# jaxonwang/k-mer-count

Hardware: AMD Instinct MI355X
Metric: k-mers/sec (whole node) on synthetic FASTA, k=31; counts bit-exact vs ref (higher is better)
Workload: dtype u64; 1 GPU; 10 GB synthetic FASTA (random_fasta_generator.py distribution, seed 2, pool 10), k=31, canonical, 1xMI355X; records_per_gpu=22371032, bases_per_gpu=8948412800, kmers_per_gpu=8277281840, kmers_all_gpus=8277281840, distinct=3350, algo=walk

## Files before the change

k-mer-count_amd/csrc/kmc_extract.hip.h:

```cpp
#pragma once
#include "kmc_stream.hip.h"
#include "kmc_msd.hip.h"

template <int KW> struct ExtractLds {
    u32 sbits[KMC_STREAM_WAVES][64];
    alignas(16) u64 tr[KMC_STREAM_WAVES][KW == 1 ? 256 : 512];
    u32 hist[KMC_MSD_NB + 3];
    u64 s_or[KMC_STREAM_WAVES][2], s_and[KMC_STREAM_WAVES][2];
};

__device__ __forceinline__ void extract_store_half(u64* tr, int lane, const u64 (&v)[8], u64* __restrict__ out_chunk, int h) {
    typedef unsigned long long u64x2_t __attribute__((ext_vector_type(2)));
#pragma unroll
    for (int q = 0; q < 4; ++q) {
        u64x2_t p = {v[2 * q], v[2 * q + 1]};
        *reinterpret_cast<u64x2_t*>(&tr[lane * 8 + 2 * ((q + (lane >> 1)) & 3)]) = p;
    }
    __builtin_amdgcn_fence(__ATOMIC_RELEASE, "wavefront");
    __builtin_amdgcn_wave_barrier();
    __builtin_amdgcn_fence(__ATOMIC_ACQUIRE, "wavefront");
    u64 x[8];
#pragma unroll
    for (int i = 0; i < 8; ++i) {
        const int l = 8 * i + (lane >> 3), j = lane & 7;
        x[i] = tr[l * 8 + 2 * (((j >> 1) + (l >> 1)) & 3) + (j & 1)];
    }
    __builtin_amdgcn_fence(__ATOMIC_RELEASE, "wavefront");
    __builtin_amdgcn_wave_barrier();
    __builtin_amdgcn_fence(__ATOMIC_ACQUIRE, "wavefront");
#pragma unroll
    for (int i = 0; i < 8; ++i) out_chunk[16 * (8 * i + (lane >> 3)) + 8 * h + (lane & 7)] = x[i];
}

template <int KW, bool CANON>
__global__ __launch_bounds__(KMC_STREAM_THREADS)
void kmc_extract_hist_kernel(const uint8_t* __restrict__ bases, u64 n_bases, const u64* __restrict__ offsets, u64 n_reads, int k,
                             u64 chunk_begin, u64 chunk_end, u64 range_begin, u32 n_ranges, u64* __restrict__ counters,
                             u64* __restrict__ out_hi, u64* __restrict__ out_lo, u32* __restrict__ hist, u32 hist_r0,
                             u64* __restrict__ rand_, u64* __restrict__ ror_) {
    constexpr int NW = 2 * KW + 1;
    extern __shared__ __align__(16) unsigned char extract_smem[];
    ExtractLds<KW>& L = *reinterpret_cast<ExtractLds<KW>*>(extract_smem);
    const int tid = threadIdx.x, lane = tid & 63, wv = tid >> 6;
    const int kb = 2 * k;
    const ChunkKeys<KW> K(k);
    const int dshift = kb > KMC_MSD_BITS ? kb - KMC_MSD_BITS : 0;
    const u32 dmask = kb >= KMC_MSD_BITS ? (u32)KMC_MSD_ND - 1u : (1u << kb) - 1u;
    u64 nk = 0;

    for (u32 r = blockIdx.x; r < n_ranges; r += gridDim.x) {
        __syncthreads();
        for (u32 d = tid; d < KMC_MSD_NB; d += KMC_STREAM_THREADS) L.hist[d] = 0;
        __syncthreads();
        u64 a_lo = ~0ull, a_hi = ~0ull, o_lo = 0, o_hi = 0;
        const u64 c0 = chunk_begin + (u64)r * (KMC_MSD_RANGE / KMC_CHUNK) + 4u * (u64)wv, c1 = c0 + 4;
        const u64 cfirst = c0 > 0 ? c0 - 1 : 0;
        ChunkWalk W(offsets, n_reads, cfirst, lane);
        for (u64 c = cfirst; c < c1; ++c) {
            W.step(bases, n_bases, c, c < chunk_end, L.sbits[wv]);
            if (c >= c0) {
                u32 X[NW], Yp[NW + 1];
                u32 inv16 = chunk_windows<KW>(W, k, X);
                if (W.pp < range_begin) {
                    const u64 nskip = range_begin - W.pp;
                    inv16 |= nskip >= 16 ? 0xFFFFu : ((1u << (u32)nskip) - 1u);
                }
                chunk_rc_stream<KW, CANON>(K, X, Yp);
                const u64 obase = W.cb - chunk_begin * KMC_CHUNK;
                auto key_at = [&](int j, u64& khi, u64& klo) -> bool {
                    chunk_key<KW, CANON>(K, X, Yp, j, khi, klo);
                    const bool ok = !((inv16 >> j) & 1);
                    const u32 d = ok ? (msd_bits<KW>(khi, klo, dshift) & dmask) : (u32)KMC_MSD_ND;
                    atomicAdd(&L.hist[d], 1u);
                    if (ok) {
                        a_lo &= klo; o_lo |= klo;
                        if constexpr (KW == 2) { a_hi &= khi; o_hi |= khi; }
                    } else {
                        klo = ~0ull; khi = ~0ull;
                    }
                    return ok;
                };
                if constexpr (KW == 1) {
                    u64 vlo[16];
#pragma unroll
                    for (int j = 0; j < 16; ++j) { u64 khi; nk += key_at(j, khi, vlo[j]) ? 1u : 0u; }
                    stream_store_transposed(reinterpret_cast<u32*>(L.tr[wv]), lane, vlo, out_lo + obase);
                } else {
#pragma unroll
                    for (int h = 0; h < 2; ++h) {
                        u64 vlo[8], vhi[8];
#pragma unroll
                        for (int j = 0; j < 8; ++j) nk += key_at(8 * h + j, vhi[j], vlo[j]) ? 1u : 0u;
                        extract_store_half(L.tr[wv], lane, vlo, out_lo + obase, h);
                        extract_store_half(L.tr[wv], lane, vhi, out_hi + obase, h);
                    }
                }
            }
        }
#pragma unroll
        for (int o = 32; o > 0; o >>= 1) {
            a_lo &= __shfl_xor(a_lo, o); o_lo |= __shfl_xor(o_lo, o);
            if (KW == 2) { a_hi &= __shfl_xor(a_hi, o); o_hi |= __shfl_xor(o_hi, o); }
        }
        if (lane == 0) { L.s_and[wv][0] = a_hi; L.s_and[wv][1] = a_lo; L.s_or[wv][0] = o_hi; L.s_or[wv][1] = o_lo; }
        __syncthreads();
        for (u32 d = tid; d < KMC_MSD_NB; d += KMC_STREAM_THREADS) hist[msd_hist_idx((size_t)hist_r0 + r, d)] = L.hist[d];
        if (tid == 0) {
            u64 ah = ~0ull, al = ~0ull, oh = 0, ol = 0;
            for (int w = 0; w < KMC_STREAM_WAVES; ++w) { ah &= L.s_and[w][0]; al &= L.s_and[w][1]; oh |= L.s_or[w][0]; ol |= L.s_or[w][1]; }
            if (KW == 1) { ah = 0; oh = 0; }
            if (KW == 1 && al == ~0ull && ol == 0) { ah = ~0ull; }
            rand_[2 * (size_t)r] = ah; rand_[2 * (size_t)r + 1] = al;
            ror_[2 * (size_t)r] = oh; ror_[2 * (size_t)r + 1] = ol;
        }
    }
    nk = wave_sum_u64(nk);
    if (lane == 0 && nk) atomicAdd((unsigned long long*)&counters[KMC_CTR_KMERS], nk);
}
```

k-mer-count_amd/csrc/kmc_msd.hip.h:

```cpp
#pragma once
#include <type_traits>
#include "kmc_device.hip.h"
#include "kmc_scan.hip.h"

#define KMC_MSD_RANGE 65536
static inline unsigned msd_range_for(unsigned long long n) {
    unsigned r = 4096;
    while (r < KMC_MSD_RANGE && (unsigned long long)r * 2048 < n) r <<= 1;
    return r;
}
#define KMC_MSD_BITS 10
#define KMC_MSD_ND (1 << KMC_MSD_BITS)
#define KMC_MSD_NB (KMC_MSD_ND + 1)
#define KMC_MSD_THREADS 256
#define KMC_MSD_LEAF1 2048
#ifndef KMC_MSD_LEAF2
#define KMC_MSD_LEAF2 2048
#endif
#define KMC_MSD_LEAF2W 1024
#ifndef KMC_MSD_THREAD_SORT
#define KMC_MSD_THREAD_SORT 32
#endif
#ifndef KMC_MSD_LEAF_LOGNSB
#define KMC_MSD_LEAF_LOGNSB 9
#endif
#define KMC_MSD_LEAF_NSB (1 << KMC_MSD_LEAF_LOGNSB)

struct MsdSeg { u32 begin, len, hib, parity; };
__device__ __forceinline__ int msd_seg_shift(u32 hib) { return hib > KMC_MSD_BITS ? (int)hib - KMC_MSD_BITS : 0; }
__device__ __forceinline__ u32 msd_seg_mask(u32 hib) { return hib >= KMC_MSD_BITS ? (u32)KMC_MSD_ND - 1u : (1u << hib) - 1u; }
struct MsdTerm { u32 begin, len, kind, parity; };
#define KMC_MSD_CNT_BITS 14

struct MsdCtl {
    u32 n_next;
    u32 n_term;
    u32 n_valid;
    u32 n_ranges;
    u32 overflow;
    u32 n_pairs;
    u32 scan_total;
    u32 pad;
    unsigned long long w_total;
    u32 n_cnt;
    u32 n_cnt2;
    u32 n_dups[64];
};

__host__ __device__ __forceinline__ size_t msd_hist_idx(size_t r, u32 d) { return ((r >> 6) * KMC_MSD_NB + d) * 64 + (r & 63); }
static inline size_t msd_hist_words(size_t n_ranges) { return ((n_ranges + 63) / 64) * 64 * (size_t)KMC_MSD_NB; }

template <int KW>
__device__ __forceinline__ bool msd_is_filler(u64 hi, u64 lo, int kb) {
    if (KW == 1) return kb < 64 && (lo >> kb) != 0;
    return (hi >> (kb - 64)) != 0;
}
template <int KW>
__device__ __forceinline__ u32 msd_bits(u64 hi, u64 lo, int shift) {
    if (KW == 1) return (u32)(lo >> shift);
    if (shift >= 64) return (u32)(hi >> (shift - 64));
    if (shift == 0) return (u32)lo;
    return (u32)((lo >> shift) | (hi << (64 - shift)));
}

__global__ __launch_bounds__(1024)
void kmc_msd_ranges_kernel(const MsdSeg* __restrict__ seg, u32 n_seg, u32 rsz, u32* __restrict__ first, MsdCtl* ctl) {
    __shared__ u32 part[1024];
    const u32 tid = threadIdx.x;
    const u32 per = (n_seg + 1023) / 1024;
    const u32 a = min(tid * per, n_seg), b = min(a + per, n_seg);
    u32 s = 0;
    for (u32 i = a; i < b; ++i) s += (seg[i].len + rsz - 1) / rsz;
    part[tid] = s;
    __syncthreads();
    for (u32 o = 1; o < 1024; o <<= 1) {
        u32 v = tid >= o ? part[tid - o] : 0;
        __syncthreads();
        part[tid] += v;
        __syncthreads();
    }
    u32 run = tid ? part[tid - 1] : 0;
    for (u32 i = a; i < b; ++i) { first[i] = run; run += (seg[i].len + rsz - 1) / rsz; }
    if (tid == 1023) { first[n_seg] = part[1023]; ctl->n_ranges = part[1023]; }
}

__device__ __forceinline__ u32 msd_seg_of(const u32* __restrict__ first, u32 n_seg, u32 r) {
    u32 lo = 0, hi = n_seg;
    while (hi - lo > 1) {
        const u32 mid = (lo + hi) >> 1;
        if (first[mid] <= r) lo = mid; else hi = mid;
    }
    return lo;
}

template <int KW>
__global__ __launch_bounds__(KMC_MSD_THREADS)
void kmc_msd_hist_kernel(const u64* __restrict__ hi0, const u64* __restrict__ lo0, const u64* __restrict__ hi1, const u64* __restrict__ lo1,
                         const MsdSeg* __restrict__ seg, u32 n_seg,
                         const u32* __restrict__ first, u32 rsz, int kb, int level0,
                         u32* __restrict__ hist, u64* __restrict__ rmin, u64* __restrict__ rmax, const MsdCtl* __restrict__ ctl) {
    __shared__ u32 h[4][KMC_MSD_NB + 3];
    __shared__ u64 smin[4][2], smax[4][2];
    const u32 r = blockIdx.x, tid = threadIdx.x, wv = tid >> 6;
    if (r >= ctl->n_ranges) return;
    for (u32 i = tid; i < 4 * (KMC_MSD_NB + 3); i += KMC_MSD_THREADS) (&h[0][0])[i] = 0;
    __syncthreads();
    const u32 s = msd_seg_of(first, n_seg, r);
    const u32 idx = r - first[s];
    const u32 b = seg[s].begin + idx * rsz;
    const u32 n = min(rsz, seg[s].len - idx * rsz);
    const int shift = msd_seg_shift(seg[s].hib);
    const u32 mask = msd_seg_mask(seg[s].hib);
    const u64* const khi = seg[s].parity ? hi1 : hi0;
    const u64* const klo = seg[s].parity ? lo1 : lo0;
    u64 mnh = ~0ull, mnl = ~0ull, mxh = 0, mxl = 0;
    for (u32 i = tid; i < n; i += KMC_MSD_THREADS) {
        const u64 lo = klo[b + i], hi = KW == 2 ? khi[b + i] : 0ull;
        u32 d;
        if (level0 && msd_is_filler<KW>(hi, lo, kb)) d = KMC_MSD_ND;
        else {
            d = msd_bits<KW>(hi, lo, shift) & mask;
            if (key_less(hi, lo, mnh, mnl)) { mnh = hi; mnl = lo; }
            if (key_less(mxh, mxl, hi, lo)) { mxh = hi; mxl = lo; }
        }
        atomicAdd(&h[wv][d], 1u);
    }
#pragma unroll
    for (int o = 32; o > 0; o >>= 1) {
        const u64 oh = __shfl_xor(mnh, o), ol = __shfl_xor(mnl, o);
        if (key_less(oh, ol, mnh, mnl)) { mnh = oh; mnl = ol; }
        const u64 ph = __shfl_xor(mxh, o), pl = __shfl_xor(mxl, o);
        if (key_less(mxh, mxl, ph, pl)) { mxh = ph; mxl = pl; }
    }
    if ((tid & 63) == 0) { smin[wv][0] = mnh; smin[wv][1] = mnl; smax[wv][0] = mxh; smax[wv][1] = mxl; }
    __syncthreads();
    for (u32 d = tid; d < KMC_MSD_NB; d += KMC_MSD_THREADS) hist[msd_hist_idx(r, d)] = h[0][d] + h[1][d] + h[2][d] + h[3][d];
    if (tid == 0) {
        for (int w = 1; w < 4; ++w) {
            if (key_less(smin[w][0], smin[w][1], mnh, mnl)) { mnh = smin[w][0]; mnl = smin[w][1]; }
            if (key_less(mxh, mxl, smax[w][0], smax[w][1])) { mxh = smax[w][0]; mxl = smax[w][1]; }
        }
        rmin[2 * (size_t)r] = mnh; rmin[2 * (size_t)r + 1] = mnl;
        rmax[2 * (size_t)r] = mxh; rmax[2 * (size_t)r + 1] = mxl;
    }
}

__global__ __launch_bounds__(KMC_MSD_THREADS)
void kmc_msd_scan_a_kernel(u32 n_seg, u32 S, const u32* __restrict__ first, u32* __restrict__ hist, u32* __restrict__ stot) {
    const u32 s = blockIdx.x / S, j = blockIdx.x % S, lane = threadIdx.x & 63, wv = threadIdx.x >> 6;
    if (s >= n_seg) return;
    const u32 r0 = first[s], r1 = first[s + 1];
    if (r1 - r0 == 1) return;
    for (u32 d = j * 4 + wv; d < KMC_MSD_NB; d += 4 * S) {
        u32 run = 0;
        for (u32 base = r0; base < r1; base += 256) {
            u32 v[4];
#pragma unroll
            for (int u = 0; u < 4; ++u) {
                const u32 r = base + 64u * u + lane;
                v[u] = r < r1 ? hist[msd_hist_idx(r, d)] : 0u;
            }
#pragma unroll
            for (int u = 0; u < 4; ++u) {
                const u32 r = base + 64u * u + lane;
                u32 inc = v[u];
#pragma unroll
                for (int o = 1; o < 64; o <<= 1) { const u32 t = __shfl_up(inc, o); if ((int)lane >= o) inc += t; }
                if (r < r1) hist[msd_hist_idx(r, d)] = run + inc - v[u];
                run += __shfl(inc, 63);
            }
        }
        if (lane == 0) stot[(size_t)s * KMC_MSD_NB + d] = run;
    }
}

__global__ __launch_bounds__(KMC_MSD_ND)
void kmc_msd_scan_kernel(const MsdSeg* __restrict__ seg, u32 n_seg, const u32* __restrict__ first, u32* __restrict__ hist, const u32* __restrict__ stot,
                         const u64* __restrict__ rmin, const u64* __restrict__ rmax, u32* __restrict__ cbase, u32* __restrict__ seg_skip,
                         int level0, int wide, u32 leaf_cap, u32 cnt_bits,
                         MsdSeg* __restrict__ next, u32 next_cap, MsdTerm* __restrict__ term, u32 term_cap,
                         unsigned long long* __restrict__ bitmap, MsdCtl* ctl) {
    constexpr int NWV = KMC_MSD_ND / 64;
    __shared__ u32 tot[KMC_MSD_NB + 7];
    __shared__ u32 cb_s[KMC_MSD_ND];
    __shared__ u32 wsum[NWV];
    __shared__ u64 smm[NWV][4];
    const u32 s = blockIdx.x, tid = threadIdx.x, lane = tid & 63, wv = tid >> 6;
    const u32 r0 = first[s], r1 = first[s + 1];
    {
        u64 mnh = ~0ull, mnl = ~0ull, mxh = 0, mxl = 0;
        for (u32 r = r0 + tid; r < r1; r += KMC_MSD_ND) {
            const u64 ah = rmin[2 * (size_t)r], al = rmin[2 * (size_t)r + 1], bh = rmax[2 * (size_t)r], bl = rmax[2 * (size_t)r + 1];
            if (key_less(ah, al, mnh, mnl)) { mnh = ah; mnl = al; }
            if (key_less(mxh, mxl, bh, bl)) { mxh = bh; mxl = bl; }
        }
#pragma unroll
        for (int o = 32; o > 0; o >>= 1) {
            const u64 oh = __shfl_xor(mnh, o), ol = __shfl_xor(mnl, o);
            if (key_less(oh, ol, mnh, mnl)) { mnh = oh; mnl = ol; }
            const u64 ph = __shfl_xor(mxh, o), pl = __shfl_xor(mxl, o);
            if (key_less(mxh, mxl, ph, pl)) { mxh = ph; mxl = pl; }
        }
        if (lane == 0) { smm[wv][0] = mnh; smm[wv][1] = mnl; smm[wv][2] = mxh; smm[wv][3] = mxl; }
    }
    if (r1 - r0 == 1) {
        for (u32 d = tid; d < KMC_MSD_NB; d += KMC_MSD_ND) { tot[d] = hist[msd_hist_idx(r0, d)]; hist[msd_hist_idx(r0, d)] = 0; }
    } else {
        for (u32 d = tid; d < KMC_MSD_NB; d += KMC_MSD_ND) tot[d] = stot[(size_t)s * KMC_MSD_NB + d];
    }
    __syncthreads();
    bool all_equal;
    int top_diff = -1;
    {
        u64 mnh = smm[0][0], mnl = smm[0][1], mxh = smm[0][2], mxl = smm[0][3];
        for (int w = 1; w < NWV; ++w) {
            if (key_less(smm[w][0], smm[w][1], mnh, mnl)) { mnh = smm[w][0]; mnl = smm[w][1]; }
            if (key_less(mxh, mxl, smm[w][2], smm[w][3])) { mxh = smm[w][2]; mxl = smm[w][3]; }
        }
        all_equal = mnh == mxh && mnl == mxl;
        const u64 xh = mnh ^ mxh, xl = mnl ^ mxl;
        if (xh) top_diff = 127 - __clzll((long long)xh);
        else if (xl) top_diff = 63 - __clzll((long long)xl);
    }
    const int shift = msd_seg_shift(seg[s].hib);
    const bool last_level = shift == 0;
    const u32 src_parity = seg[s].parity;
    const u32 n_filler = level0 ? tot[KMC_MSD_ND] : 0;
    const bool equal = all_equal && seg[s].len > n_filler && (!level0 || n_filler == 0);
    const u32 mine = tot[tid];
    u32 inc = mine;
#pragma unroll
    for (int o = 1; o < 64; o <<= 1) { const u32 v = __shfl_up(inc, o); if ((int)lane >= o) inc += v; }
    if (lane == 63) wsum[wv] = inc;
    __syncthreads();
    u32 wbase = 0;
    for (u32 w = 0; w < wv; ++w) wbase += wsum[w];
    const u32 cb = seg[s].begin + wbase + inc - mine;
    cbase[(size_t)s * KMC_MSD_NB + tid] = cb;
    cb_s[tid] = cb;
    __syncthreads();
    __shared__ u32 l_tb[KMC_MSD_ND], l_tl[KMC_MSD_ND], l_tk[KMC_MSD_ND], l_nb[KMC_MSD_ND], l_nl[KMC_MSD_ND];
    const bool nomove = !equal && !last_level && top_diff >= 0 && top_diff < shift && n_filler == 0;
    if (wv != 0 && (!wide || equal || nomove)) return;
    const u32 lb = wide ? wv * 64u : 0u;
    if (tid == 0) {
        cbase[(size_t)s * KMC_MSD_NB + KMC_MSD_ND] = 0;
        seg_skip[s] = (equal || nomove) ? 1u : 0u;
        if (level0) ctl->n_valid = seg[s].len - n_filler;
    }
    u32 nt = 0, nn = 0, ncnt = 0;
    u32 q_hib = (u32)shift, q_par = src_parity ^ 1u, t_par = src_parity ^ 1u;
    if (equal) {
        if (lane == 0) { l_tb[0] = seg[s].begin; l_tl[0] = seg[s].len; l_tk[0] = 1u; }
        nt = 1; t_par = src_parity;
    } else if (nomove && cnt_bits && (u32)(top_diff + 1) <= cnt_bits && seg[s].len > leaf_cap) {
        if (lane == 0) { l_tb[0] = seg[s].begin; l_tl[0] = seg[s].len; l_tk[0] = 2u | ((u32)(top_diff + 1) << 8); }
        nt = 1; ncnt = 1; t_par = src_parity;
    } else if (nomove) {
        if (lane == 0) { l_nb[0] = seg[s].begin; l_nl[0] = seg[s].len; }
        nn = 1; q_hib = (u32)(top_diff + 1); q_par = src_parity;
    } else {
        u32 gb = 0, gl = 0;
        auto flush = [&]() { if (lane == 0) { l_tb[lb + nt] = gb; l_tl[lb + nt] = gl; l_tk[lb + nt] = gl == 1 ? 1u : 0u; } ++nt; gl = 0; };
        const int jb = wide ? (int)wv : 0, je = wide ? (int)wv + 1 : NWV;
        for (int j = jb; j < je; ++j) {
            const u32 Tj = tot[j * 64 + lane], Cj = cb_s[j * 64 + lane];
            unsigned long long live = __builtin_amdgcn_ballot_w64(Tj != 0);
            while (live) {
                const int bl = (int)__builtin_ctzll(live);
                live &= live - 1;
                const u32 m = (u32)__builtin_amdgcn_readlane((int)Tj, bl);
                const u32 cbv = (u32)__builtin_amdgcn_readlane((int)Cj, bl);
                if (m > leaf_cap) {
                    if (gl) flush();
                    if (last_level) { if (lane == 0) { l_tb[lb + nt] = cbv; l_tl[lb + nt] = m; l_tk[lb + nt] = 1u; } ++nt; }
                    else if (cnt_bits && (u32)shift <= cnt_bits) {
                        if (lane == 0) { l_tb[lb + nt] = cbv; l_tl[lb + nt] = m; l_tk[lb + nt] = 2u | ((u32)shift << 8); }
                        ++nt; ++ncnt;
                    }
                    else { if (lane == 0) { l_nb[lb + nn] = cbv; l_nl[lb + nn] = m; } ++nn; }
                } else {
                    if (gl && gl + m > leaf_cap) flush();
                    if (!gl) gb = cbv;
                    gl += m;
                }
            }
        }
        if (gl) flush();
    }
    u32 t_base = 0, n_base = 0;
    if (lane == 0) {
        if (nt) { t_base = atomicAdd(&ctl->n_term, nt); if (t_base + nt > term_cap) atomicOr(&ctl->overflow, 1u); }
        if (nn) { n_base = atomicAdd(&ctl->n_next, nn); if (n_base + nn > next_cap) atomicOr(&ctl->overflow, 2u); }
        if (ncnt) atomicAdd(&ctl->n_cnt, ncnt);
    }
    t_base = (u32)__builtin_amdgcn_readfirstlane((int)t_base);
    n_base = (u32)__builtin_amdgcn_readfirstlane((int)n_base);
    __builtin_amdgcn_fence(__ATOMIC_RELEASE, "wavefront");
    __builtin_amdgcn_wave_barrier();
    __builtin_amdgcn_fence(__ATOMIC_ACQUIRE, "wavefront");
    for (u32 i = lane; i < nt; i += 64) {
        if (t_base + i >= term_cap) break;
        const u32 bg = l_tb[lb + i];
        term[t_base + i] = MsdTerm{bg, l_tl[lb + i], l_tk[lb + i], t_par};
        atomicOr(&bitmap[bg >> 6], 1ull << (bg & 63));
    }
    for (u32 i = lane; i < nn; i += 64) {
        if (n_base + i >= next_cap) break;
        next[n_base + i] = MsdSeg{l_nb[lb + i], l_nl[lb + i], q_hib, q_par};
    }
}

#ifdef KMC_LEAF_STAMPS
__device__ unsigned long long kmc_leaf_stamps[16];
#define LEAF_STAMP(i) do { __syncthreads(); if (threadIdx.x == 0) { const unsigned long long now_ = __builtin_amdgcn_s_memtime(); atomicAdd(&kmc_leaf_stamps[i], now_ - t_prev_); t_prev_ = __builtin_amdgcn_s_memtime(); } } while (0)
#else
#define LEAF_STAMP(i) do { } while (0)
#endif
template <int KW, bool WEIGHTS> struct MsdScatterLds {
    static constexpr int WORDS = KW + (WEIGHTS ? 1 : 0);
    static constexpr int TILE = WORDS == 1 ? 16384 : (WORDS == 2 ? 8192 : 4096);
    u64 lo[TILE];
    u64 hi[KW == 2 ? TILE : 1];
    u64 w[WEIGHTS ? TILE : 1];
    u32 cnt[KMC_MSD_NB + 3];
    u32 gdst[KMC_MSD_NB + 3];
    u32 cur[KMC_MSD_NB + 3];
    u32 wsum[16];
};
template <int KW, bool WEIGHTS>
__global__ __launch_bounds__(1024)
void kmc_msd_scatter_kernel(u64* __restrict__ hi0, u64* __restrict__ lo0, u64* __restrict__ w0,
                            u64* __restrict__ hi1, u64* __restrict__ lo1, u64* __restrict__ w1,
                            const MsdSeg* __restrict__ seg, u32 n_seg, const u32* __restrict__ first, u32 rsz,
                            const u32* __restrict__ hist, const u32* __restrict__ cbase, const u32* __restrict__ seg_skip,
                            int kb, int level0, const MsdCtl* __restrict__ ctl) {
    extern __shared__ __align__(16) unsigned char msd_smem[];
    typedef MsdScatterLds<KW, WEIGHTS> LT;
    LT& L = *reinterpret_cast<LT*>(msd_smem);
    constexpr int TILE = LT::TILE, PER = TILE / 1024;
    const u32 r = blockIdx.x, tid = threadIdx.x, lane = tid & 63, wv = tid >> 6;
    if (r >= ctl->n_ranges) return;
    const u32 s = msd_seg_of(first, n_seg, r);
    if (seg_skip[s]) return;
    const int shift = msd_seg_shift(seg[s].hib);
    const u32 mask = msd_seg_mask(seg[s].hib);
    const bool sp = seg[s].parity != 0;
    const u64* const khi = sp ? hi1 : hi0;
    const u64* const klo = sp ? lo1 : lo0;
    const u64* const kw = sp ? w1 : w0;
    u64* const ohi = sp ? hi0 : hi1;
    u64* const olo = sp ? lo0 : lo1;
    u64* const ow = sp ? w0 : w1;
    for (u32 d = tid; d < KMC_MSD_NB; d += 1024) L.cur[d] = cbase[(size_t)s * KMC_MSD_NB + d] + hist[msd_hist_idx(r, d)];
    const u32 idx = r - first[s];
    const u32 b = seg[s].begin + idx * rsz;
    const u32 n = min(rsz, seg[s].len - idx * rsz);
    static_assert(PER % 2 == 0, "keys per thread must be even");
    typedef unsigned long long u64x2_t __attribute__((ext_vector_type(2)));
    const u32 off = b & 1u;
    u64 nlo[PER], nhi[PER], nw[PER];
    auto load_tile = [&](u32 t0, u32 tn) {
#pragma unroll
        for (int e = 0; e < PER / 2; ++e) {
            const u32 s0 = 2u * (tid + 1024u * e);
            if (s0 + off < tn) {
                const size_t g = (size_t)b + t0 + off + s0;
                const u64x2_t pl = *reinterpret_cast<const u64x2_t*>(klo + g);
                nlo[2 * e] = pl.x; nlo[2 * e + 1] = pl.y;
                if (KW == 2) { const u64x2_t ph = *reinterpret_cast<const u64x2_t*>(khi + g); nhi[2 * e] = ph.x; nhi[2 * e + 1] = ph.y; }
                if (WEIGHTS) { const u64x2_t pw = *reinterpret_cast<const u64x2_t*>(kw + g); nw[2 * e] = pw.x; nw[2 * e + 1] = pw.y; }
            }
            if (off) {
#pragma unroll
                for (int h = 0; h < 2; ++h) {
                    if (s0 + h == tn - 1) {
                        nlo[2 * e + h] = klo[(size_t)b + t0];
                        if (KW == 2) nhi[2 * e + h] = khi[(size_t)b + t0];
                        if (WEIGHTS) nw[2 * e + h] = kw[(size_t)b + t0];
                    }
                }
            }
        }
    };
#pragma unroll
    for (int e = 0; e < PER; ++e) { nlo[e] = 0; nhi[e] = 0; nw[e] = 0; }
    load_tile(0, min((u32)TILE, n));
#ifdef KMC_LEAF_STAMPS
    unsigned long long t_prev_ = __builtin_amdgcn_s_memtime();
#endif
    for (u32 t0 = 0; t0 < n; t0 += TILE) {
        const u32 tn = min((u32)TILE, n - t0);
        for (u32 d = tid; d < KMC_MSD_NB; d += 1024) L.cnt[d] = 0;
        __syncthreads();
        LEAF_STAMP(8);
        u64 mlo[PER], mhi[PER], mw[PER];
        u32 md[PER];
#pragma unroll
        for (int e = 0; e < PER; ++e) {
            md[e] = ~0u;
            mlo[e] = nlo[e]; mhi[e] = nhi[e]; mw[e] = nw[e];
            if (2u * (tid + 1024u * (e >> 1)) + (e & 1) < tn) {
                const u32 d = (level0 && msd_is_filler<KW>(mhi[e], mlo[e], kb)) ? (u32)KMC_MSD_ND : (msd_bits<KW>(mhi[e], mlo[e], shift) & mask);
                md[e] = d | (atomicAdd(&L.cnt[d], 1u) << 11);
            }
        }
        if (t0 + TILE < n) load_tile(t0 + TILE, min((u32)TILE, n - t0 - TILE));
        __syncthreads();
        LEAF_STAMP(9);
        {
            const u32 c = L.cnt[tid];
            u32 inc = c;
#pragma unroll
            for (int o = 1; o < 64; o <<= 1) { const u32 v = __shfl_up(inc, o); if ((int)lane >= o) inc += v; }
            if (lane == 63) L.wsum[wv] = inc;
            __syncthreads();
            u32 base = 0;
            for (u32 w = 0; w < wv; ++w) base += L.wsum[w];
            const u32 off = base + inc - c;
            L.cnt[tid] = off;
            L.gdst[tid] = L.cur[tid] - off;
            L.cur[tid] += c;
            if (tid == 1023) L.cnt[KMC_MSD_ND] = off + c;
        }
        __syncthreads();
        LEAF_STAMP(10);
#pragma unroll
        for (int e = 0; e < PER; ++e) {
            if (md[e] != ~0u) {
                const u32 p = L.cnt[md[e] & 2047u] + (md[e] >> 11);
                L.lo[p] = mlo[e];
                if (KW == 2) L.hi[p] = mhi[e];
                if (WEIGHTS) L.w[p] = mw[e];
            }
        }
        __syncthreads();
        LEAF_STAMP(11);
        const u32 n_keys = L.cnt[KMC_MSD_ND];
#pragma unroll
        for (int e = 0; e < PER; ++e) {
            const u32 p = tid + 1024u * e;
            if (p < n_keys) {
                const u64 lo = L.lo[p], hi = KW == 2 ? L.hi[p] : 0ull;
                const u32 d = msd_bits<KW>(hi, lo, shift) & mask;
                const u32 q = L.gdst[d] + p;
                olo[q] = lo;
                if (KW == 2) ohi[q] = hi;
                if (WEIGHTS) ow[q] = L.w[p];
            }
        }
        __syncthreads();
        LEAF_STAMP(12);
    }
}

__global__ void kmc_msd_order_kernel(const MsdTerm* __restrict__ term, u32 n_term, const unsigned long long* __restrict__ bitmap,
                                     const u32* __restrict__ rank, MsdTerm* __restrict__ ordered, u32* __restrict__ clist, MsdCtl* ctl) {
    for (u32 i = blockIdx.x * blockDim.x + threadIdx.x; i < n_term; i += gridDim.x * blockDim.x) {
        const u32 p = term[i].begin;
        const unsigned long long below = bitmap[p >> 6] & ((1ull << (p & 63)) - 1ull);
        const u32 o = rank[p >> 6] + (u32)__popcll(below);
        ordered[o] = term[i];
        if ((term[i].kind & 0xFFu) == 2u) clist[atomicAdd(&ctl->n_cnt2, 1u)] = o;
    }
}

template <int KW>
__global__ __launch_bounds__(1024)
void kmc_msd_count_kernel(const u64* __restrict__ hi0, const u64* __restrict__ lo0, const u64* __restrict__ hi1, const u64* __restrict__ lo1,
                          const MsdTerm* __restrict__ term, const u32* __restrict__ clist, u32 n_list,
                          u64* __restrict__ o_hi, u64* __restrict__ o_lo, u64* __restrict__ o_cnt, u32* __restrict__ nd, MsdCtl* __restrict__ ctl) {
    __shared__ u32 cnt[1u << KMC_MSD_CNT_BITS];
    __shared__ u32 wsum[16];
    const u32 tid = threadIdx.x, lane = tid & 63, wv = tid >> 6;
    if (blockIdx.x >= n_list) return;
    const u32 t = clist[blockIdx.x];
    const MsdTerm T = term[t];
    const u32 bits = T.kind >> 8, nbin = 1u << bits, n = T.len;
    const u64 mask = (u64)nbin - 1ull;
    const u64* const klo = (T.parity ? lo1 : lo0) + T.begin;
    for (u32 i = tid; i < nbin; i += 1024) cnt[i] = 0;
    __syncthreads();
    u32 i = tid;
    for (; i + 3 * 1024 < n; i += 4 * 1024) {
        const u64 a = klo[i], b = klo[i + 1024], c = klo[i + 2048], d = klo[i + 3072];
        atomicAdd(&cnt[(u32)(a & mask)], 1u); atomicAdd(&cnt[(u32)(b & mask)], 1u);
        atomicAdd(&cnt[(u32)(c & mask)], 1u); atomicAdd(&cnt[(u32)(d & mask)], 1u);
    }
    for (; i < n; i += 1024) atomicAdd(&cnt[(u32)(klo[i] & mask)], 1u);
    const u64 plo = klo[0] & ~mask;
    const u64 phi = KW == 2 ? ((T.parity ? hi1 : hi0)[T.begin]) : 0ull;
    __syncthreads();
    const u32 per = nbin >= 1024 ? nbin / 1024 : 1u;
    const u32 b0 = tid * per;
    u32 mine = 0;
    if (b0 < nbin) for (u32 e = 0; e < per; ++e) mine += cnt[b0 + e] ? 1u : 0u;
    u32 inc = mine;
#pragma unroll
    for (int o = 1; o < 64; o <<= 1) { const u32 v = __shfl_up(inc, o); if ((int)lane >= o) inc += v; }
    if (lane == 63) wsum[wv] = inc;
    __syncthreads();
    u32 base = 0, total = 0;
    for (u32 w = 0; w < 16; ++w) { if (w < wv) base += wsum[w]; total += wsum[w]; }
    u32 r = T.begin + base + inc - mine;
    if (b0 < nbin) for (u32 e = 0; e < per; ++e) {
        const u32 c = cnt[b0 + e];
        if (c) { o_lo[r] = plo | (u64)(b0 + e); if (KW == 2) o_hi[r] = phi; o_cnt[r] = c; ++r; }
    }
    if (tid == 0) {
        nd[t] = total;
        if (total != n) atomicAdd(&ctl->n_dups[t & 63u], n - total);
    }
}


template <int KW, bool WEIGHTS, int CAPV, int SCRV> struct MsdLeafLds {
    static constexpr int CAP = CAPV;
    u64 b_lo[CAP];
    u64 b_hi[KW == 2 ? CAP : 1];
    u64 b_w[WEIGHTS ? CAP : 1];
    static constexpr int SCR = SCRV;
    u64 s_lo[4][SCR];
    u64 s_hi[KW == 2 ? 4 : 1][KW == 2 ? SCR : 1];
    u64 s_w[WEIGHTS ? 4 : 1][WEIGHTS ? SCR : 1];
    u32 cnt[KMC_MSD_LEAF_NSB], off[KMC_MSD_LEAF_NSB + 1];
    u32 big[CAPV / (KMC_MSD_THREAD_SORT + 1) + 2];
    u32 woff[4][129];
    u32 nbig;
    u32 wsum[4];
    u32 bad;
    u32 n_out;
    u64 sx[4][2], sy[4][2];
};

template <int KW, bool WEIGHTS, int CAPV, int SCRV>
__global__ __launch_bounds__(KMC_MSD_THREADS, (KW == 1 && !WEIGHTS) ? 7 : 1)
void kmc_msd_leaf_kernel(const u64* __restrict__ hi0, const u64* __restrict__ lo0, const u64* __restrict__ w0,
                         const u64* __restrict__ hi1, const u64* __restrict__ lo1, const u64* __restrict__ w1,
                         const MsdTerm* __restrict__ term, u32 n_term, int kb,
                         u64* __restrict__ s_hi0, u64* __restrict__ s_lo0, u64* __restrict__ s_w0,
                         u64* __restrict__ s_hi1, u64* __restrict__ s_lo1, u64* __restrict__ s_w1,
                         u64* __restrict__ o_hi, u64* __restrict__ o_lo, u64* __restrict__ o_cnt,
                         u32* __restrict__ nd, MsdCtl* __restrict__ ctl) {
    extern __shared__ __align__(16) unsigned char msd_smem[];
    MsdLeafLds<KW, WEIGHTS, CAPV, SCRV>& L = *reinterpret_cast<MsdLeafLds<KW, WEIGHTS, CAPV, SCRV>*>(msd_smem);
    const u32 t = blockIdx.x, tid = threadIdx.x, lane = tid & 63, wv = tid >> 6;
    const MsdTerm T = term[t];
    const u64* khi = T.parity ? hi1 : hi0;
    const u64* klo = T.parity ? lo1 : lo0;
    const u64* kw = T.parity ? w1 : w0;
    u64* const t_lo = T.parity ? s_lo0 : s_lo1;
    u64* const t_hi = T.parity ? s_hi0 : s_hi1;
    u64* const t_w = T.parity ? s_w0 : s_w1;
    const u32 n = T.len;
#ifdef KMC_LEAF_STAMPS
    unsigned long long t_prev_ = __builtin_amdgcn_s_memtime();
#endif
    auto account = [&](u32 n_mine) {
        nd[t] = n_mine;
        if (n_mine != n) atomicAdd(&ctl->n_dups[t & 63u], n - n_mine);
    };
    auto single_pair = [&](u64 hi, u64 lo, u64 cnt, u32 n_mine) {
        if (tid == 0) {
            account(n_mine);
            if (n_mine) {
                o_lo[T.begin] = lo; if (KW == 2) o_hi[T.begin] = hi; o_cnt[T.begin] = cnt;
                if (WEIGHTS) atomicAdd(&ctl->w_total, (unsigned long long)cnt);
            }
        }
    };
    if ((T.kind & 0xFFu) == 2u) return;
    if (T.kind == 1) {
        u64 s = n;
        if (WEIGHTS) {
            s = 0;
            for (u32 i = tid; i < n; i += KMC_MSD_THREADS) s += kw[T.begin + i];
            s = wave_sum_u64(s);
            if (lane == 0) L.sx[wv][0] = s;
            __syncthreads();
            s = L.sx[0][0] + L.sx[1][0] + L.sx[2][0] + L.sx[3][0];
        }
        single_pair(KW == 2 ? khi[T.begin] : 0ull, klo[T.begin], s, 1u);
        return;
    }
    constexpr int PER = MsdLeafLds<KW, WEIGHTS, CAPV, SCRV>::CAP / KMC_MSD_THREADS;
    u64 rlo[PER], rhi[KW == 2 ? PER : 1], rw[WEIGHTS ? PER : 1];
    u64 mnh = ~0ull, mnl = ~0ull, mxh = 0, mxl = 0;
    static_assert(PER % 2 == 0, "keys per thread must be even");
    typedef unsigned long long u64x2_t __attribute__((ext_vector_type(2)));
    const u32 off = T.begin & 1u;
    bool rv[PER];
#pragma unroll
    for (int e = 0; e < PER / 2; ++e) {
        const u32 s0 = 2u * (tid + KMC_MSD_THREADS * e);
        rlo[2 * e] = rlo[2 * e + 1] = 0;
        if (KW == 2) rhi[2 * e] = rhi[2 * e + 1] = 0;
        if (WEIGHTS) rw[2 * e] = rw[2 * e + 1] = 0;
        rv[2 * e] = s0 + off < n;
        rv[2 * e + 1] = s0 + 1 + off < n;
        if (rv[2 * e]) {
            const size_t g = (size_t)T.begin + off + s0;
            const u64x2_t pl = *reinterpret_cast<const u64x2_t*>(klo + g);
            rlo[2 * e] = pl.x; rlo[2 * e + 1] = pl.y;
            if (KW == 2) { const u64x2_t ph = *reinterpret_cast<const u64x2_t*>(khi + g); rhi[2 * e] = ph.x; rhi[2 * e + 1] = ph.y; }
            if (WEIGHTS) { const u64x2_t pw = *reinterpret_cast<const u64x2_t*>(kw + g); rw[2 * e] = pw.x; rw[2 * e + 1] = pw.y; }
        }
        if (off) {
#pragma unroll
            for (int h = 0; h < 2; ++h) {
                if (s0 + h == n - 1) {
                    rlo[2 * e + h] = klo[T.begin];
                    if (KW == 2) rhi[2 * e + h] = khi[T.begin];
                    if (WEIGHTS) rw[2 * e + h] = kw[T.begin];
                    rv[2 * e + h] = true;
                }
            }
        }
    }
#pragma unroll
    for (int e = 0; e < PER; ++e) {
        if (rv[e]) {
            const u64 lo = rlo[e], hi = KW == 2 ? rhi[e] : 0ull;
            if (key_less(hi, lo, mnh, mnl)) { mnh = hi; mnl = lo; }
            if (key_less(mxh, mxl, hi, lo)) { mxh = hi; mxl = lo; }
        } else {
            rlo[e] = 0;
            if (KW == 2) rhi[e] = 0;
            if (WEIGHTS) rw[e] = 0;
        }
    }
    LEAF_STAMP(0);
    for (u32 i = tid; i < KMC_MSD_LEAF_NSB; i += KMC_MSD_THREADS) L.cnt[i] = 0;
    if (tid == 0) { L.bad = 0; L.n_out = 0; L.nbig = 0; }
#pragma unroll
    for (int o = 32; o > 0; o >>= 1) {
        const u64 oh = __shfl_xor(mnh, o), ol = __shfl_xor(mnl, o);
        if (key_less(oh, ol, mnh, mnl)) { mnh = oh; mnl = ol; }
        const u64 ph = __shfl_xor(mxh, o), pl = __shfl_xor(mxl, o);
        if (key_less(mxh, mxl, ph, pl)) { mxh = ph; mxl = pl; }
    }
    if (lane == 0) { L.sx[wv][0] = mnh; L.sx[wv][1] = mnl; L.sy[wv][0] = mxh; L.sy[wv][1] = mxl; }
    __syncthreads();
    mnh = L.sx[0][0]; mnl = L.sx[0][1]; mxh = L.sy[0][0]; mxl = L.sy[0][1];
    for (int w = 1; w < 4; ++w) {
        if (key_less(L.sx[w][0], L.sx[w][1], mnh, mnl)) { mnh = L.sx[w][0]; mnl = L.sx[w][1]; }
        if (key_less(mxh, mxl, L.sy[w][0], L.sy[w][1])) { mxh = L.sy[w][0]; mxl = L.sy[w][1]; }
    }
    const u64 fh = mnh, fl = mnl;
    const u64 rl = mxl - mnl, rh = mxh - mnh - (mxl < mnl ? 1ull : 0ull);
    const int top = rh ? 127 - __clzll((long long)rh) : (rl ? 63 - __clzll((long long)rl) : -1);
    if (top < 0) {
        u64 sw = n;
        if (WEIGHTS) {
            __syncthreads();
            sw = 0;
#pragma unroll
            for (int e = 0; e < PER; ++e) if (rv[e]) sw += rw[e];
            sw = wave_sum_u64(sw);
            if (lane == 0) L.sx[wv][0] = sw;
            __syncthreads();
            sw = L.sx[0][0] + L.sx[1][0] + L.sx[2][0] + L.sx[3][0];
        }
        single_pair(fh, fl, sw, n ? 1u : 0u);
        return;
    }
    const int shift = top >= KMC_MSD_LEAF_LOGNSB ? top - (KMC_MSD_LEAF_LOGNSB - 1) : 0;
    auto bucket = [&](u64 hi, u64 lo) -> u32 {
        const u64 dl = lo - mnl;
        if (KW == 1) return (u32)(dl >> shift);
        const u64 dh = hi - mnh - (lo < mnl ? 1ull : 0ull);
        if (shift >= 64) return (u32)(dh >> (shift - 64));
        if (shift == 0) return (u32)dl;
        return (u32)((dl >> shift) | (dh << (64 - shift)));
    };
    LEAF_STAMP(1);
    u32 rb[PER];
#pragma unroll
    for (int e = 0; e < PER; ++e) {
        rb[e] = bucket(KW == 2 ? rhi[e] : 0ull, rlo[e]) & (KMC_MSD_LEAF_NSB - 1u);
        if (rv[e]) atomicAdd(&L.cnt[rb[e]], 1u);
    }
    __syncthreads();
    {
        constexpr int PT = KMC_MSD_LEAF_NSB / KMC_MSD_THREADS;
        u32 c[PT], mine = 0;
#pragma unroll
        for (int e = 0; e < PT; ++e) { c[e] = L.cnt[tid * PT + e]; mine += c[e]; }
        u32 inc = mine;
#pragma unroll
        for (int o = 1; o < 64; o <<= 1) { const u32 v = __shfl_up(inc, o); if ((int)lane >= o) inc += v; }
        if (lane == 63) L.wsum[wv] = inc;
        __syncthreads();
        u32 run = inc - mine;
        for (u32 w = 0; w < wv; ++w) run += L.wsum[w];
#pragma unroll
        for (int e = 0; e < PT; ++e) {
            L.off[tid * PT + e] = run;
            L.cnt[tid * PT + e] = run;
            if (c[e] > KMC_MSD_THREAD_SORT) L.big[atomicAdd(&L.nbig, 1u)] = tid * PT + e;
            run += c[e];
        }
        if (tid == KMC_MSD_THREADS - 1) L.off[KMC_MSD_LEAF_NSB] = run;
        __syncthreads();
    }
    LEAF_STAMP(2);
    u32 rp[PER];
#pragma unroll
    for (int e = 0; e < PER; ++e) {
        rp[e] = 0;
        if (rv[e]) {
            const u32 p = atomicAdd(&L.cnt[rb[e]], 1u);
            rp[e] = p;
            L.b_lo[p] = rlo[e];
            if (KW == 2) L.b_hi[p] = rhi[e];
            if (WEIGHTS) L.b_w[p] = rw[e];
        }
    }
    __syncthreads();
    LEAF_STAMP(3);
#ifdef KMC_EXP_INSERTION
    for (int e = 0; e < PER; ++e) rp[e] = ~0u;
    for (u32 d = tid * (KMC_MSD_LEAF_NSB / KMC_MSD_THREADS); d < (tid + 1) * (KMC_MSD_LEAF_NSB / KMC_MSD_THREADS); ++d) {
        const u32 o = L.off[d], m = L.off[d + 1] - o;
        if (m > 1 && m <= KMC_MSD_THREAD_SORT) {
            for (u32 i = 1; i < m; ++i) {
                const u64 lo = L.b_lo[o + i], hi = KW == 2 ? L.b_hi[o + i] : 0ull;
                u64 w = 0;
                if (WEIGHTS) w = L.b_w[o + i];
                u32 j = i;
                while (j > 0) {
                    const u64 pl = L.b_lo[o + j - 1], ph = KW == 2 ? L.b_hi[o + j - 1] : 0ull;
                    if (!key_less(hi, lo, ph, pl)) break;
                    L.b_lo[o + j] = pl;
                    if (KW == 2) L.b_hi[o + j] = ph;
                    if (WEIGHTS) L.b_w[o + j] = L.b_w[o + j - 1];
                    --j;
                }
                if (j != i) {
                    L.b_lo[o + j] = lo;
                    if (KW == 2) L.b_hi[o + j] = hi;
                    if (WEIGHTS) L.b_w[o + j] = w;
                }
            }
        }
    }
#else
#pragma unroll
    for (int e = 0; e < PER; ++e) {
        if (rv[e]) {
            const u32 o = L.off[rb[e]], m = L.off[rb[e] + 1] - o;
            if (m > 1 && m <= KMC_MSD_THREAD_SORT) {
                const u64 mlo = rlo[e], mhi = KW == 2 ? rhi[e] : 0ull;
                const u32 mp = rp[e];
                u32 rank = 0;
                for (u32 j = 0; j < m; ++j) {
                    const u64 ql = L.b_lo[o + j], qh = KW == 2 ? L.b_hi[o + j] : 0ull;
                    const bool before = key_less(qh, ql, mhi, mlo) || (qh == mhi && ql == mlo && o + j < mp);
                    rank += before ? 1u : 0u;
                }
                rp[e] = o + rank;
            } else {
                rp[e] = ~0u;
            }
        } else rp[e] = ~0u;
    }
#endif
    __syncthreads();
#pragma unroll
    for (int e = 0; e < PER; ++e) {
        if (rp[e] != ~0u) {
            L.b_lo[rp[e]] = rlo[e];
            if (KW == 2) L.b_hi[rp[e]] = rhi[e];
            if (WEIGHTS) L.b_w[rp[e]] = rw[e];
        }
    }
    __syncthreads();
    LEAF_STAMP(4);
    auto allpairs = [&](const u64* s_lo, const u64* s_hi, const u64* s_w, u64* d_lo, u64* d_hi, u64* d_w, u32 m) {
        for (u32 c = 0; c < m; c += 64) {
            const u32 i = c + lane;
            u64 lo = 0, hi = 0, w = 0;
            const bool have = i < m;
            if (have) { lo = s_lo[i]; if (KW == 2) hi = s_hi[i]; if (WEIGHTS) w = s_w[i]; }
            u32 rk = 0;
            for (u32 e = 0; e < m; e += 64) {
                const u32 j = e + lane;
                u64 ql = ~0ull, qh = ~0ull;
                if (j < m) { ql = s_lo[j]; qh = KW == 2 ? s_hi[j] : 0ull; }
                const u32 mm = min(64u, m - e);
                for (u32 x = 0; x < mm; ++x) {
                    const u64 ol = ((u64)(u32)__builtin_amdgcn_readlane((int)(u32)(ql >> 32), (int)x) << 32) | (u32)__builtin_amdgcn_readlane((int)(u32)ql, (int)x);
                    u64 oh = 0;
                    if (KW == 2) oh = ((u64)(u32)__builtin_amdgcn_readlane((int)(u32)(qh >> 32), (int)x) << 32) | (u32)__builtin_amdgcn_readlane((int)(u32)qh, (int)x);
                    const bool less = key_less(oh, ol, hi, lo);
                    const bool eq = oh == hi && ol == lo;
                    rk += (less || (eq && (e + x) < i)) ? 1u : 0u;
                }
            }
            if (have) { d_lo[rk] = lo; if (KW == 2) d_hi[rk] = hi; if (WEIGHTS) d_w[rk] = w; }
        }
    };
    u64* const g_lo = t_lo + T.begin;
    u64* const g_hi = KW == 2 ? t_hi + T.begin : nullptr;
    u64* const g_w = WEIGHTS ? t_w + T.begin : nullptr;
    const u32 nbig = L.nbig;
    for (u32 bi = wv; bi < nbig; bi += 4) {
        const u32 d = L.big[bi];
        const u32 o = L.off[d], m = L.off[d + 1] - o;
        u64 mnh = ~0ull, mnl = ~0ull, mxh = 0, mxl = 0;
        for (u32 i = lane; i < m; i += 64) {
            const u64 lo = L.b_lo[o + i], hi = KW == 2 ? L.b_hi[o + i] : 0ull;
            if (key_less(hi, lo, mnh, mnl)) { mnh = hi; mnl = lo; }
            if (key_less(mxh, mxl, hi, lo)) { mxh = hi; mxl = lo; }
        }
#pragma unroll
        for (int s2 = 32; s2 > 0; s2 >>= 1) {
            const u64 oh = __shfl_xor(mnh, s2), ol = __shfl_xor(mnl, s2);
            if (key_less(oh, ol, mnh, mnl)) { mnh = oh; mnl = ol; }
            const u64 ph = __shfl_xor(mxh, s2), pl = __shfl_xor(mxl, s2);
            if (key_less(mxh, mxl, ph, pl)) { mxh = ph; mxl = pl; }
        }
        if (mnh == mxh && mnl == mxl) continue;
        const u64 rl2 = mxl - mnl, rh2 = mxh - mnh - (mxl < mnl ? 1ull : 0ull);
        const int top2 = rh2 ? 127 - __clzll((long long)rh2) : 63 - __clzll((long long)rl2);
        const int sh2 = top2 >= 7 ? top2 - 6 : 0;
        auto bkt2 = [&](u64 hi, u64 lo) -> u32 {
            const u64 dl = lo - mnl;
            if (KW == 1) return (u32)(dl >> sh2) & 127u;
            const u64 dh = hi - mnh - (lo < mnl ? 1ull : 0ull);
            if (sh2 >= 64) return (u32)(dh >> (sh2 - 64)) & 127u;
            if (sh2 == 0) return (u32)dl & 127u;
            return (u32)((dl >> sh2) | (dh << (64 - sh2))) & 127u;
        };
        constexpr u32 SCR = (u32)MsdLeafLds<KW, WEIGHTS, CAPV, SCRV>::SCR;
        const bool use_g = m > SCR;
        const u32 xo = use_g ? 0u : o;
        u64* const x_lo = use_g ? g_lo : &L.s_lo[wv][0];
        u64* const x_hi = KW == 2 ? (use_g ? g_hi : &L.s_hi[wv][0]) : nullptr;
        u64* const x_w = WEIGHTS ? (use_g ? g_w : &L.s_w[wv][0]) : nullptr;
        auto xsync = [&]() {
            if (use_g) {
                __builtin_amdgcn_fence(__ATOMIC_RELEASE, "agent");
                __builtin_amdgcn_wave_barrier();
                __builtin_amdgcn_fence(__ATOMIC_ACQUIRE, "agent");
            } else {
                __builtin_amdgcn_fence(__ATOMIC_RELEASE, "wavefront");
                __builtin_amdgcn_wave_barrier();
                __builtin_amdgcn_fence(__ATOMIC_ACQUIRE, "wavefront");
            }
        };
        u32* const wc = &L.cnt[wv * 128];
        u32* const wo = L.woff[wv];
#pragma unroll
        for (int e = 0; e < 2; ++e) wc[lane * 2 + e] = 0;
        xsync();
        for (u32 i = lane; i < m; i += 64) atomicAdd(&wc[bkt2(KW == 2 ? L.b_hi[o + i] : 0ull, L.b_lo[o + i])], 1u);
        xsync();
        {
            u32 c4[2], mine = 0;
#pragma unroll
            for (int e = 0; e < 2; ++e) { c4[e] = wc[lane * 2 + e]; mine += c4[e]; }
            u32 inc = mine;
#pragma unroll
            for (int s2 = 1; s2 < 64; s2 <<= 1) { const u32 v = __shfl_up(inc, s2); if ((int)lane >= s2) inc += v; }
            u32 run = inc - mine;
#pragma unroll
            for (int e = 0; e < 2; ++e) { wo[lane * 2 + e] = run; wc[lane * 2 + e] = run; run += c4[e]; }
            if (lane == 63) wo[128] = run;
        }
        xsync();
        for (u32 i = lane; i < m; i += 64) {
            const u64 lo = L.b_lo[o + i], hi = KW == 2 ? L.b_hi[o + i] : 0ull;
            const u32 pp = atomicAdd(&wc[bkt2(hi, lo)], 1u);
            x_lo[(o + pp) - xo] = lo;
            if (KW == 2) x_hi[(o + pp) - xo] = hi;
            if (WEIGHTS) x_w[(o + pp) - xo] = L.b_w[o + i];
        }
        xsync();
        u32 big_mask = 0;
#pragma unroll
        for (int e = 0; e < 2; ++e) {
            const u32 oo = o + wo[lane * 2 + e], mm = wo[lane * 2 + e + 1] - wo[lane * 2 + e];
            if (mm > KMC_MSD_THREAD_SORT) { big_mask |= 1u << e; continue; }
            for (u32 i = 1; i < mm; ++i) {
                const u64 lo = x_lo[(oo + i) - xo], hi = KW == 2 ? x_hi[(oo + i) - xo] : 0ull;
                u64 w = 0;
                if (WEIGHTS) w = x_w[(oo + i) - xo];
                u32 j = i;
                while (j > 0) {
                    const u64 pl = x_lo[(oo + j - 1) - xo], ph = KW == 2 ? x_hi[(oo + j - 1) - xo] : 0ull;
                    if (!key_less(hi, lo, ph, pl)) break;
                    x_lo[(oo + j) - xo] = pl;
                    if (KW == 2) x_hi[(oo + j) - xo] = ph;
                    if (WEIGHTS) x_w[(oo + j) - xo] = x_w[(oo + j - 1) - xo];
                    --j;
                }
                if (j != i) { x_lo[(oo + j) - xo] = lo; if (KW == 2) x_hi[(oo + j) - xo] = hi; if (WEIGHTS) x_w[(oo + j) - xo] = w; }
            }
        }
        xsync();
        unsigned long long todo;
        while ((todo = __builtin_amdgcn_ballot_w64(big_mask != 0)) != 0) {
            const int src_lane = (int)__builtin_ctzll(todo);
            const u32 bm = (u32)__builtin_amdgcn_readlane((int)big_mask, src_lane);
            const int e = __ffs((int)bm) - 1;
            const u32 oo = o + wo[src_lane * 2 + e];
            const u32 mm = wo[src_lane * 2 + e + 1] - wo[src_lane * 2 + e];
            if ((int)lane == src_lane) big_mask &= ~(1u << e);
            const u64 plo = x_lo[(oo) - xo], phi = KW == 2 ? x_hi[(oo) - xo] : 0ull;
            bool diff = false;
            for (u32 i = lane; i < mm; i += 64) diff |= x_lo[(oo + i) - xo] != plo || (KW == 2 && x_hi[(oo + i) - xo] != phi);
            if (__builtin_amdgcn_ballot_w64(diff) == 0) continue;
            if (mm > 1024) { if (lane == 0) L.bad = 1; continue; }
            allpairs(x_lo + (oo - xo), KW == 2 ? x_hi + (oo - xo) : nullptr, WEIGHTS ? x_w + (oo - xo) : nullptr,
                     &L.b_lo[oo], KW == 2 ? &L.b_hi[oo] : nullptr, WEIGHTS ? &L.b_w[oo] : nullptr, mm);
            xsync();
            for (u32 i = lane; i < mm; i += 64) { x_lo[(oo + i) - xo] = L.b_lo[oo + i]; if (KW == 2) x_hi[(oo + i) - xo] = L.b_hi[oo + i]; if (WEIGHTS) x_w[(oo + i) - xo] = L.b_w[oo + i]; }
            xsync();
        }
        for (u32 i = lane; i < m; i += 64) {
            L.b_lo[o + i] = x_lo[(o + i) - xo];
            if (KW == 2) L.b_hi[o + i] = x_hi[(o + i) - xo];
            if (WEIGHTS) L.b_w[o + i] = x_w[(o + i) - xo];
        }
    }
    __syncthreads();
    if (L.bad) {
        u32 P = 1;
        while (P < n) P <<= 1;
        for (u32 i = n + tid; i < P; i += KMC_MSD_THREADS) {
            L.b_lo[i] = ~0ull;
            if (KW == 2) L.b_hi[i] = ~0ull;
            if (WEIGHTS) L.b_w[i] = 0ull;
        }
        __syncthreads();
        for (u32 kk = 2; kk <= P; kk <<= 1) {
            for (u32 jj = kk >> 1; jj > 0; jj >>= 1) {
                for (u32 i = tid; i < P; i += KMC_MSD_THREADS) {
                    const u32 ix = i ^ jj;
                    if (ix > i) {
                        const u64 al = L.b_lo[i], bl = L.b_lo[ix];
                        const u64 ah = KW == 2 ? L.b_hi[i] : 0ull, bh = KW == 2 ? L.b_hi[ix] : 0ull;
                        const bool up = (i & kk) == 0;
                        const bool sw = up ? key_less(bh, bl, ah, al) : key_less(ah, al, bh, bl);
                        if (sw) {
                            L.b_lo[i] = bl; L.b_lo[ix] = al;
                            if (KW == 2) { L.b_hi[i] = bh; L.b_hi[ix] = ah; }
                            if (WEIGHTS) { const u64 wa = L.b_w[i]; L.b_w[i] = L.b_w[ix]; L.b_w[ix] = wa; }
                        }
                    }
                }
                __syncthreads();
            }
        }
    }
    LEAF_STAMP(5);
    static_assert(sizeof(L.cnt) + sizeof(L.off) >= MsdLeafLds<KW, WEIGHTS, CAPV, SCRV>::CAP * sizeof(unsigned short), "run-head list does not fit");
    unsigned short* const hidx = reinterpret_cast<unsigned short*>(L.cnt);
    constexpr int NSLAB = MsdLeafLds<KW, WEIGHTS, CAPV, SCRV>::CAP / KMC_MSD_THREADS;
    u32 hmask = 0;
    u32 hpre[NSLAB];
    u32* const stot = L.big;
    static_assert(sizeof(L.big) >= (NSLAB * 4 + 1) * sizeof(u32), "head totals do not fit");
#pragma unroll
    for (int e = 0; e < NSLAB; ++e) {
        const u32 i = tid + KMC_MSD_THREADS * e;
        bool h = false;
        if (i < n) h = i == 0 || L.b_lo[i] != L.b_lo[i - 1] || (KW == 2 && L.b_hi[i] != L.b_hi[i - 1]);
        const unsigned long long m = __builtin_amdgcn_ballot_w64(h);
        hmask |= h ? (1u << e) : 0u;
        hpre[e] = __builtin_amdgcn_mbcnt_hi((u32)(m >> 32), __builtin_amdgcn_mbcnt_lo((u32)m, 0u));
        if (lane == 0) stot[e * 4 + wv] = (u32)__popcll(m);
    }
    __syncthreads();
    u32 n_heads = 0;
    {
        static_assert(NSLAB * 4 <= 64, "one wave scans the head totals");
        if (wv == 0) {
            const u32 v = lane < NSLAB * 4 ? stot[lane] : 0u;
            u32 inc = v;
#pragma unroll
            for (int o = 1; o < 64; o <<= 1) { const u32 x = __shfl_up(inc, o); if ((int)lane >= o) inc += x; }
            if (lane < NSLAB * 4) stot[lane] = inc - v;
            if (lane == NSLAB * 4 - 1) stot[NSLAB * 4] = inc;
        }
        __syncthreads();
        n_heads = stot[NSLAB * 4];
#pragma unroll
        for (int e = 0; e < NSLAB; ++e) if (hmask & (1u << e)) hidx[stot[e * 4 + wv] + hpre[e]] = (unsigned short)(tid + KMC_MSD_THREADS * e);
    }
    __syncthreads();
    LEAF_STAMP(6);
    const u32 n_out = n_heads;
    if (tid == 0) account(n_out);
    const u32 base = T.begin;
    u64 wtot = 0;
    auto pair_of = [&](u32 r, u64& khi_o, u64& klo_o, u64& c_o) {
        const u32 i = hidx[r], iend = r + 1 < n_out ? hidx[r + 1] : n;
        u64 sum = iend - i;
        if (WEIGHTS) { sum = 0; for (u32 j = i; j < iend; ++j) sum += L.b_w[j]; }
        klo_o = L.b_lo[i];
        khi_o = KW == 2 ? L.b_hi[i] : 0ull;
        c_o = sum;
        wtot += sum;
    };
    const u32 lead = (base & 1u) && n_out ? 1u : 0u;
    if (tid == 0 && lead) {
        u64 a, b, cn;
        pair_of(0, a, b, cn);
        o_lo[base] = b; if (KW == 2) o_hi[base] = a; o_cnt[base] = cn;
    }
    for (u32 r = lead + 2u * tid; r < n_out; r += 2u * KMC_MSD_THREADS) {
        u64 h0, l0, c0, h1 = 0, l1 = 0, c1 = 0;
        pair_of(r, h0, l0, c0);
        if (r + 1 < n_out) {
            pair_of(r + 1, h1, l1, c1);
            const size_t g = (size_t)base + r;
            *reinterpret_cast<u64x2_t*>(o_lo + g) = u64x2_t{l0, l1};
            if (KW == 2) *reinterpret_cast<u64x2_t*>(o_hi + g) = u64x2_t{h0, h1};
            *reinterpret_cast<u64x2_t*>(o_cnt + g) = u64x2_t{c0, c1};
        } else {
            o_lo[base + r] = l0; if (KW == 2) o_hi[base + r] = h0; o_cnt[base + r] = c0;
        }
    }
    if (WEIGHTS) {
        wtot = wave_sum_u64(wtot);
        if (lane == 0 && wtot) atomicAdd(&ctl->w_total, (unsigned long long)wtot);
    }
    LEAF_STAMP(7);
}

template <int KW>
__global__ void kmc_msd_gather_kernel(const MsdTerm* __restrict__ term, u32 n_term, const u32* __restrict__ nd, const u32* __restrict__ base,
                                      const u64* __restrict__ s_hi, const u64* __restrict__ s_lo, const u64* __restrict__ s_cnt,
                                      u64* __restrict__ o_hi, u64* __restrict__ o_lo, u64* __restrict__ o_cnt) {
    const u32 wave = (blockIdx.x * blockDim.x + threadIdx.x) >> 6, lane = threadIdx.x & 63, n_waves = (gridDim.x * blockDim.x) >> 6;
    for (u32 t = wave; t < n_term; t += n_waves) {
        const u32 src = term[t].begin, dst = base[t], m = nd[t];
        for (u32 i = lane; i < m; i += 64) {
            o_lo[dst + i] = s_lo[src + i];
            if (KW == 2) o_hi[dst + i] = s_hi[src + i];
            o_cnt[dst + i] = s_cnt[src + i];
        }
    }
}
```

Before: 6210 billion k-mers/s.

## Widen LDS transpose for KW=1 extract stores and vectorize MSD histogram loads

For single-word keys, the extract kernel now writes each key straight into a larger 16-slot-per-lane LDS tile with a rotated, bank-spreading index. It then reads the tile back so each global store is a fully coalesced 64-lane row, replacing the old stream_store_transposed path. The MSD histogram kernel now loads keys as 128-bit pairs, with two pairs per thread per iteration, handling an odd start and tail separately to cut load instruction count. The cost is four times more LDS per wave for KW=1, which may lower occupancy, and the pair loop can read one element past the segment end when the count is odd.

```diff
diff --git a/k-mer-count_amd/csrc/kmc_extract.hip.h b/k-mer-count_amd/csrc/kmc_extract.hip.h
--- a/k-mer-count_amd/csrc/kmc_extract.hip.h
+++ b/k-mer-count_amd/csrc/kmc_extract.hip.h
@@ -4,10 +4,28 @@
 
 template <int KW> struct ExtractLds {
     u32 sbits[KMC_STREAM_WAVES][64];
-    alignas(16) u64 tr[KMC_STREAM_WAVES][KW == 1 ? 256 : 512];
+    alignas(16) u64 tr[KMC_STREAM_WAVES][KW == 1 ? 1024 : 512];
     u32 hist[KMC_MSD_NB + 3];
     u64 s_or[KMC_STREAM_WAVES][2], s_and[KMC_STREAM_WAVES][2];
 };
+
+__device__ __forceinline__ u32 extract_tr_slot(int lane, int j) { return (u32)(lane * 16 + ((j + lane) & 15)); }
+__device__ __forceinline__ void extract_store_rows(const u64* tr, int lane, u64* __restrict__ out_chunk) {
+    __builtin_amdgcn_fence(__ATOMIC_RELEASE, "wavefront");
+    __builtin_amdgcn_wave_barrier();
+    __builtin_amdgcn_fence(__ATOMIC_ACQUIRE, "wavefront");
+#pragma unroll
+    for (int g = 0; g < 2; ++g) {
+        u64 x[8];
+#pragma unroll
+        for (int i = 0; i < 8; ++i) x[i] = tr[extract_tr_slot(4 * (8 * g + i) + (lane >> 4), lane & 15)];
+#pragma unroll
+        for (int i = 0; i < 8; ++i) out_chunk[(8 * g + i) * 64 + lane] = x[i];
+    }
+    __builtin_amdgcn_fence(__ATOMIC_RELEASE, "wavefront");
+    __builtin_amdgcn_wave_barrier();
+    __builtin_amdgcn_fence(__ATOMIC_ACQUIRE, "wavefront");
+}
 
 __device__ __forceinline__ void extract_store_half(u64* tr, int lane, const u64 (&v)[8], u64* __restrict__ out_chunk, int h) {
     typedef unsigned long long u64x2_t __attribute__((ext_vector_type(2)));
@@ -81,10 +99,13 @@
                     return ok;
                 };
                 if constexpr (KW == 1) {
-                    u64 vlo[16];
 #pragma unroll
-                    for (int j = 0; j < 16; ++j) { u64 khi; nk += key_at(j, khi, vlo[j]) ? 1u : 0u; }
-                    stream_store_transposed(reinterpret_cast<u32*>(L.tr[wv]), lane, vlo, out_lo + obase);
+                    for (int j = 0; j < 16; ++j) {
+                        u64 khi, klo;
+                        nk += key_at(j, khi, klo) ? 1u : 0u;
+                        L.tr[wv][extract_tr_slot(lane, j)] = klo;
+                    }
+                    extract_store_rows(L.tr[wv], lane, out_lo + obase);
                 } else {
 #pragma unroll
                     for (int h = 0; h < 2; ++h) {
diff --git a/k-mer-count_amd/csrc/kmc_msd.hip.h b/k-mer-count_amd/csrc/kmc_msd.hip.h
--- a/k-mer-count_amd/csrc/kmc_msd.hip.h
+++ b/k-mer-count_amd/csrc/kmc_msd.hip.h
@@ -114,8 +114,7 @@
     const u64* const khi = seg[s].parity ? hi1 : hi0;
     const u64* const klo = seg[s].parity ? lo1 : lo0;
     u64 mnh = ~0ull, mnl = ~0ull, mxh = 0, mxl = 0;
-    for (u32 i = tid; i < n; i += KMC_MSD_THREADS) {
-        const u64 lo = klo[b + i], hi = KW == 2 ? khi[b + i] : 0ull;
+    auto count = [&](u64 hi, u64 lo) {
         u32 d;
         if (level0 && msd_is_filler<KW>(hi, lo, kb)) d = KMC_MSD_ND;
         else {
@@ -124,6 +123,28 @@
             if (key_less(mxh, mxl, hi, lo)) { mxh = hi; mxl = lo; }
         }
         atomicAdd(&h[wv][d], 1u);
+    };
+    typedef unsigned long long u64x2_t __attribute__((ext_vector_type(2)));
+    const u32 off = b & 1u;
+    if (off && tid == 0) count(KW == 2 ? khi[b] : 0ull, klo[b]);
+    const u32 m = n - off;
+    const u32 np = (m + 1) / 2;
+    const size_t g0 = (size_t)b + off;
+    for (u32 p = tid; p < np; p += 2 * KMC_MSD_THREADS) {
+        const u32 p1 = p + KMC_MSD_THREADS;
+        const bool two = p1 < np;
+        u64x2_t l0 = *reinterpret_cast<const u64x2_t*>(klo + g0 + 2 * (size_t)p), l1 = {0, 0}, h0 = {0, 0}, h1 = {0, 0};
+        if (KW == 2) h0 = *reinterpret_cast<const u64x2_t*>(khi + g0 + 2 * (size_t)p);
+        if (two) {
+            l1 = *reinterpret_cast<const u64x2_t*>(klo + g0 + 2 * (size_t)p1);
+            if (KW == 2) h1 = *reinterpret_cast<const u64x2_t*>(khi + g0 + 2 * (size_t)p1);
+        }
+        count(h0.x, l0.x);
+        if (2 * p + 1 < m) count(h0.y, l0.y);
+        if (two) {
+            count(h1.x, l1.x);
+            if (2 * p1 + 1 < m) count(h1.y, l1.y);
+        }
     }
 #pragma unroll
     for (int o = 32; o > 0; o >>= 1) {
```

New measurement: 6223 billion k-mers/s (median of 3 runs). Within noise of the previous version (+0.2%).
